# miaoyin390/DNN-Compression-Tensor-ADMM

Measured on AMD Instinct MI355X. Metric: ADMM projection iters/sec (all layers) + per-layer SVD GFLOP/s, ResNet-50 TT ranks, higher is better.
Workload: dtype f32 (Gram, eigen-solve and its filter products accumulate in f64); 1 GPU; resnet50_tt: 34 layers, 20099072 weights, hp table tt_resnet50_hp.HyperParamsDictGeneralRatio3x; tables=1, parallelism=layer-shard x1 (latency-model partition, one scalar all-reduce per step)

## Files before the change

### dnn-compression-tensor-admm_amd/csrc/common.h

```cpp
#pragma once
#include <hip/hip_runtime.h>
#include <stdint.h>
#include <stddef.h>
#include "../../include/tadmm.h"

namespace tadmm {

constexpr int kWave = 64;

struct BlockRef { int32_t prob; int32_t local; };

struct SweepDesc {
  const float* W; float* U; float* Z;
  float* T0;
  const float* Zmat;
  int32_t O, I, K2;
  int32_t ichunk;
  int32_t nchunk;
  int64_t numel;
  int32_t blk_begin;
  int32_t nblk;
};

void launch_unfold(const SweepDesc* descs_dev, const BlockRef* map_dev, int nblocks, int use_u, hipStream_t s);
void launch_fold_update(const SweepDesc* descs_dev, const BlockRef* map_dev, int nblocks, int update_u,
                        double* resid_partial_dev, hipStream_t s);
void launch_resid_reduce(const SweepDesc* descs_dev, int nlayers, const double* resid_partial_dev,
                         double* resid_sq_dev, hipStream_t s, const int32_t* out_index = nullptr);

struct GramDesc {
  const float* A;
  int32_t m, n;
  int32_t trans;
  int32_t N, K;
  int32_t nt;
  int32_t ksplit, kchunk;
  double* partial;
  double* G;
  int32_t Npad, ld;
};
void launch_gram_partial(const GramDesc* descs_dev, const BlockRef* map_dev, int nblocks, hipStream_t s,
                         const int32_t* skip = nullptr);
void launch_gram_reduce(const GramDesc* descs_dev, const BlockRef* map_dev, int nblocks, hipStream_t s,
                        const int32_t* skip = nullptr);

constexpr int kJB = 8;
struct EigDesc {
  double* XT;
  int32_t N, Npad, ld, nb;
  double* off;
  int32_t* done;
  double* lam;
  int32_t* order;
  double* sigma;
  int32_t r;
  int32_t mode;
  float* out_a;
  float* out_b;
  double* evec_out;
  double* sblk;
  int32_t ldo;
  double* warm;
  int32_t* warm_ok;
  double* scratch;
  int32_t period;
};
void launch_jacobi_init(const EigDesc* descs_dev, int nprob, hipStream_t s, const int32_t* skip = nullptr,
                        double* prev_dev = nullptr);
void launch_jacobi_conv(const EigDesc* descs_dev, int nprob, int tick, double tol, bool super, double* prev_dev,
                        int* verdict_pinned, hipStream_t s);
constexpr int kJacobiMaxN = 8160;
bool jacobi_size_supported(int n);
size_t jacobi_tick_stream_lds_bytes();
size_t jacobi_tick_lds_bytes(int ld_max);
size_t jacobi_tick2_lds_bytes(int ld_max);
bool jacobi_tick2_fits(int ld_max);
hipError_t launch_jacobi_tick(const EigDesc* descs_dev, const BlockRef* map_dev, int nblocks, int tick, double tol,
                              int inner_sweeps, size_t lds_bytes, bool super, hipStream_t s);
void dump_stamps();
size_t jacobi_tick3_lds_bytes(int ld_max);
bool jacobi_tick3_fits(int ld_max);
hipError_t launch_jacobi_tick3(const EigDesc* descs_dev, const BlockRef* map_dev, int nblocks, int tick, double tol,
                               int ld_max, hipStream_t s);
constexpr int kLdResidentMax = 1152;
static inline int eig_ld(int N) { return (N + 127) / 128 * 128; }
hipError_t launch_jacobi_self(const EigDesc* descs_dev, const BlockRef* map_dev, int nblocks, int tick, double tol,
                              int inner_sweeps, int ld_max, hipStream_t s);
bool jacobi_small_fits(int npad_max);
hipError_t launch_jacobi_small(const EigDesc* descs_dev, int nprob, int npad_max, double tol, int max_sweeps,
                               const int32_t* skip, int* verdict_pinned, hipStream_t s, bool warm,
                               const int32_t* fast_done = nullptr);
bool eig_small_direct_on();
bool eig_mid_direct_on();
bool eig_mid_direct_size(int n);
size_t eig_mid_scratch_bytes(int n);
void launch_eig_mid_direct(const EigDesc* descs_dev, int nprob, int ns, const int32_t* skip, int* verdict_pinned, hipStream_t s);
hipError_t launch_eig_small_direct(const EigDesc* descs_dev, int nprob, const int32_t* skip, int32_t* fast_done_dev,
                                   int* verdict_pinned, hipStream_t s);
void launch_eig_norms(const EigDesc* descs_dev, const BlockRef* map_dev, int nblocks, hipStream_t s,
                      const int32_t* skip = nullptr);
void launch_eig_sort(const EigDesc* descs_dev, int nprob, hipStream_t s, const int32_t* skip = nullptr, int npad_max = 0);
void launch_eig_extract(const EigDesc* descs_dev, const BlockRef* map_dev, int nblocks, hipStream_t s,
                        const int32_t* skip = nullptr);

struct GemmDesc {
  const float* A; const float* B; float* C;
  int32_t M, N, K;
  int64_t a_rs, a_cs, b_rs, b_cs, c_rs, c_cs;
  float alpha, beta;
  const float* bias_n; const float* bias_m;
  int32_t tiles_m, tiles_n;
};
constexpr int kGemmBM = 64, kGemmBN = 64;
void launch_gemm(const GemmDesc* descs_dev, const BlockRef* map_dev, int nblocks, hipStream_t s,
                 const int32_t* skip = nullptr);
void launch_gemm_one(const GemmDesc& d, hipStream_t s);
void launch_gemm_bf16_nt(const void* A, const void* Bt, void* C, int M, int N, int K, int64_t lda, int64_t ldb,
                         int64_t ldc, const float* bias_n, hipStream_t s);

#if defined(__HIP_DEVICE_COMPILE__) || defined(__HIPCC__)
template <typename T> using G = T __attribute__((address_space(1)));
template <typename T> __device__ __forceinline__ G<T>* gp(T* p) { return (G<T>*)p; }
#endif

struct ChainDesc {
  const void* X; void* Y;
  const uint16_t* Win; const uint16_t* Wout;
  const float* bias;
  int64_t T;
  int32_t Kin, R, Nout;
  int64_t ldx, ldy, win_plane, wout_plane;
  int32_t x_hw, y_hw, x_vec, y_vec, fused;
  long long* stamps;
  void* H;
  int64_t ldh;
  int32_t rt, h_vec;
};
int launch_tt_chain(const ChainDesc& d, int dtype, int tile_tokens, hipStream_t s);
int launch_svdconv_chain(const ChainDesc& d, int dtype, int tile_tokens, hipStream_t s);

struct ConvChainDesc {
  const void* X; void* Y;
  const uint16_t* W1; const uint16_t* W2; const uint16_t* W3;
  const float* bias;
  int64_t w1_plane, w2_plane, w3_plane;
  int32_t B, C, R1, R2, Nout;
  int32_t H, W, Ho, Wo, kh, kw, sh, sw, ph, pw, dh, dw;
  int32_t TM, TR, tiles, NT;
  int32_t x_vec;
  int32_t transposed;
  void* S1; void* S2;
  int32_t r1t, r2t;
};
int launch_tt_conv(const ConvChainDesc& d, int dtype, hipStream_t s);
bool plan_tt_conv(ConvChainDesc& d, int dtype, size_t* lds_bytes);

struct DgemmDesc {
  const double* A; const double* B; const double* C;
  const double* P; const double* Q;
  double* ring[3];
  const int32_t* rot;
  int32_t selA, selB, selC, selP, selQ;
  int32_t M, N, K;
  int32_t lda, ldb, ldc;
  int32_t tiles_m, tiles_n;
  int32_t mode;
  const double* coef;
  const double* theta;
  double* rowpart;
  const int32_t* gate; int32_t gate_min;
  const uint16_t* Gp; int64_t g_plane;
};
void launch_dgemm(const DgemmDesc* descs_dev, const BlockRef* map_dev, int nblocks, bool b_transposed, hipStream_t s);
void launch_dgemm_nt64(const DgemmDesc* descs_dev, const BlockRef* map_dev, int nblocks, hipStream_t s, int tile_n = 64,
                       int tile_m = 64);
void launch_daxpby(const DgemmDesc* descs_dev, const BlockRef* map_dev, int nblocks, hipStream_t s);
struct GPlaneDesc {
  const double* Gm; int32_t ldg;
  int32_t nt, ks;
  uint16_t* out; int64_t plane;
};
void launch_gplanes(const GPlaneDesc* descs_dev, const BlockRef* map_dev, int nblocks, hipStream_t s);
void launch_dgemm3(const DgemmDesc* descs_dev, const BlockRef* map_dev, int nblocks, hipStream_t s);

constexpr int kCholStrip = 16;
struct CholDesc {
  const double* C; int32_t ldc;
  int32_t n;
  double* R; int32_t ldr;
  double* Wd;
  double* ring[3]; const int32_t* rot; int32_t sel;
  int32_t ldy, ncols;
  int32_t* bad;
  const int32_t* gate; int32_t gate_min;
  int32_t* rot_out;
};
void launch_chol_factor(const CholDesc* descs_dev, int nprob, hipStream_t s);
void launch_chol_solve(const CholDesc* descs_dev, const BlockRef* map_dev, int nblocks, hipStream_t s);

struct FiltState {
  int32_t base, res;
  int32_t nsteps;
  int32_t active;
  int32_t alive;
  int32_t bad;
  int32_t stage;
  int32_t products;
  int32_t products_fast;
  int32_t precise_stages;
  double logamp;
  double logamp_precise;
  double coef1[2];
  double coefk[3];
  double b, lr, l1;
  double crit;
  double guard;
  double mom[64 * 5];
  int32_t mom_on;
};
struct FiltProb {
  FiltState* st;
  double* ring[3];
  int32_t N, Npad, rp, r, r32;
  int32_t ldy;
  const double* rqpart; int32_t rq_tiles;
  const double* vpart; int32_t v_tiles;
  const double* lam; const int32_t* order;
  double* sigma;
  double* theta;
  const double* UT;
  int32_t mode, ldo;
  float* out_a; float* out_b;
  int32_t* skip_slot;
  int32_t* fb_skip;
  const double* G; int32_t ldg;
  const double* H; int32_t ldh;
};
struct FiltParams {
  int32_t max_degree;
  double log_target;
  double cond_max;
  double cond_first;
  double sin_tol;
  double log_precise;
};
struct CompDesc {
  FiltState* st;
  const double* G; double* Gc;
  int32_t N, Npad, ldg;
  double* cshift;
  const double* UT; int32_t ldy, k;
  double* Cimg; int32_t r;
  float* out_a; int32_t ldo;
  double* sigma_layer;
};
void launch_comp_prepare(const CompDesc* descs_dev, int nprob, int npad_max, int steps, hipStream_t s);
void launch_comp_form(const CompDesc* descs_dev, const BlockRef* map_dev, int nblocks, hipStream_t s);
void launch_comp_emit(const CompDesc* descs_dev, const BlockRef* map_dev, int nblocks, hipStream_t s);
void launch_filt_init(const FiltProb* probs_dev, const BlockRef* map_dev, int nblocks, int nprob, hipStream_t s);
void launch_filt_guard(const FiltProb* probs_dev, int nprob, int npad_max, int rp_max, int steps, hipStream_t s);
void launch_filt_moments(const FiltProb* probs_dev, int nprob, hipStream_t s);
void launch_filt_plan(const FiltProb* probs_dev, int nprob, FiltParams prm, int last_stage, int stage_fast, int* verdict_pinned,
                      hipStream_t s);
void launch_filt_flags(const FiltProb* probs_dev, int nprob, hipStream_t s);
void launch_filt_theta(const FiltProb* probs_dev, int nprob, hipStream_t s);
void launch_filt_verdict(const FiltProb* probs_dev, int nprob, FiltParams prm, int* verdict_pinned, hipStream_t s);
void launch_filt_emit(const FiltProb* probs_dev, const BlockRef* map_dev, int nblocks, hipStream_t s);

constexpr int kPenaltyBlocks = 1024;
void launch_penalty(int n, const void* const* ptrs_dev, const int64_t* numel_dev, int64_t total, float rho,
                    float gscale, double* loss_dev, double* partial_dev, hipStream_t s);

}
```

### dnn-compression-tensor-admm_amd/csrc/gemm.hip

```cpp
#include "common.h"

namespace tadmm {

typedef float float16_t __attribute__((ext_vector_type(16)));

constexpr int BM = kGemmBM, BN = kGemmBN, BK = 16;
constexpr int LDA = BM + 4, LDB = BN + 4;

struct Frag4 { float v[4]; };

__device__ __forceinline__ Frag4 load_tile4(const float* __restrict__ P, int64_t rs, int64_t cs, bool kcontig,
                                            int row0, int nrows, int k0, int K, int tid) {
  Frag4 f;
  if (kcontig) {
    const int rr = tid >> 2, kk = (tid & 3) * 4;
    const int row = row0 + rr;
    const bool rok = row < nrows;
    const float* p = P + (int64_t)row * rs + (int64_t)(k0 + kk) * cs;
    if (rok && (k0 + kk + 3) < K && ((((uintptr_t)p) & 15) == 0)) {
      const float4 t = *reinterpret_cast<const float4*>(p);
      f.v[0] = t.x; f.v[1] = t.y; f.v[2] = t.z; f.v[3] = t.w;
    } else {
#pragma unroll
      for (int e = 0; e < 4; ++e) f.v[e] = (rok && (k0 + kk + e) < K) ? p[e] : 0.f;
    }
  } else {
    const int kk = tid >> 4, rr = (tid & 15) * 4;
    const int k = k0 + kk;
    const bool kok = k < K;
    const float* p = P + (int64_t)(row0 + rr) * rs + (int64_t)k * cs;
    if (kok && (row0 + rr + 3) < nrows && ((((uintptr_t)p) & 15) == 0)) {
      const float4 t = *reinterpret_cast<const float4*>(p);
      f.v[0] = t.x; f.v[1] = t.y; f.v[2] = t.z; f.v[3] = t.w;
    } else {
#pragma unroll
      for (int e = 0; e < 4; ++e) f.v[e] = (kok && (row0 + rr + e) < nrows) ? p[e] : 0.f;
    }
  }
  return f;
}

__device__ __forceinline__ void store_tile4(float* __restrict__ S, int ldS, bool kcontig, const Frag4& f, int tid) {
  if (kcontig) {
    const int rr = tid >> 2, kk = (tid & 3) * 4;
#pragma unroll
    for (int e = 0; e < 4; ++e) S[(kk + e) * ldS + rr] = f.v[e];
  } else {
    const int kk = tid >> 4, rr = (tid & 15) * 4;
    *reinterpret_cast<float4*>(&S[kk * ldS + rr]) = make_float4(f.v[0], f.v[1], f.v[2], f.v[3]);
  }
}

template <bool kComp>
__device__ __forceinline__ void gemm_tile(const GemmDesc& d, int local, float* __restrict__ As, float* __restrict__ Bs) {
  const int tm = local / d.tiles_n, tn = local - tm * d.tiles_n;
  const int m0 = tm * BM, n0 = tn * BN;
  const int tid = threadIdx.x, lane = tid & 63, wave = tid >> 6;
  const int wm = wave >> 1, wn = wave & 1;
  const bool a_k = (d.a_cs == 1), b_k = (d.b_rs == 1) && (d.b_cs != 1);
  const int K = d.K;
  const float16_t zero16 = {0, 0, 0, 0, 0, 0, 0, 0, 0, 0, 0, 0, 0, 0, 0, 0};
  float16_t acc0 = zero16, tot = zero16;

  Frag4 fa = load_tile4(d.A, d.a_rs, d.a_cs, a_k, m0, d.M, 0, K, tid);
  Frag4 fb = load_tile4(d.B, d.b_cs, d.b_rs, b_k, n0, d.N, 0, K, tid);
  const int ai = wm * 32 + (lane & 31), bj = wn * 32 + (lane & 31), kq = lane >> 5;
  int chunk = 0;
  for (int k0 = 0; k0 < K; k0 += BK) {
    store_tile4(As, LDA, a_k, fa, tid);
    store_tile4(Bs, LDB, b_k, fb, tid);
    __syncthreads();
    if (k0 + BK < K) {
      fa = load_tile4(d.A, d.a_rs, d.a_cs, a_k, m0, d.M, k0 + BK, K, tid);
      fb = load_tile4(d.B, d.b_cs, d.b_rs, b_k, n0, d.N, k0 + BK, K, tid);
    }
#pragma unroll
    for (int kk = 0; kk < BK; kk += 2) {
      const float a = As[(kk + kq) * LDA + ai];
      const float b = Bs[(kk + kq) * LDB + bj];
      acc0 = __builtin_amdgcn_mfma_f32_32x32x2f32(a, b, acc0, 0, 0, 0);
    }
    if (kComp && ++chunk == 4) {
      chunk = 0;
#pragma unroll
      for (int e = 0; e < 16; ++e) tot[e] += acc0[e];
      acc0 = zero16;
    }
    __syncthreads();
  }
  float16_t acc;
#pragma unroll
  for (int e = 0; e < 16; ++e) acc[e] = kComp ? tot[e] + acc0[e] : acc0[e];

  const int col = n0 + wn * 32 + (lane & 31);
  if (col < d.N) {
    const float bn = d.bias_n ? d.bias_n[col] : 0.f;
#pragma unroll
    for (int reg = 0; reg < 16; ++reg) {
      const int row = m0 + wm * 32 + (reg & 3) + 8 * (reg >> 2) + 4 * (lane >> 5);
      if (row < d.M) {
        float* c = d.C + (int64_t)row * d.c_rs + (int64_t)col * d.c_cs;
        float v = d.alpha * acc[reg] + bn;
        if (d.bias_m) v += d.bias_m[row];
        if (d.beta != 0.f) v += d.beta * (*c);
        *c = v;
      }
    }
  }
}

template <bool kComp>
__global__ __launch_bounds__(256) void gemm_kernel(const GemmDesc* __restrict__ descs,
                                                   const BlockRef* __restrict__ map,
                                                   const int32_t* __restrict__ skip) {
  __shared__ __attribute__((aligned(16))) float As[BK * LDA];
  __shared__ __attribute__((aligned(16))) float Bs[BK * LDB];
  const BlockRef br = map[blockIdx.x];
  if (skip && skip[br.prob]) return;
  const GemmDesc d = descs[br.prob];
  gemm_tile<kComp>(d, br.local, As, Bs);
}

template <bool kComp>
__global__ __launch_bounds__(256) void gemm_one_kernel(const GemmDesc d) {
  __shared__ __attribute__((aligned(16))) float As[BK * LDA];
  __shared__ __attribute__((aligned(16))) float Bs[BK * LDB];
  gemm_tile<kComp>(d, blockIdx.x, As, Bs);
}

static bool gemm_plain() {
  const char* e = getenv("TADMM_GEMM_PLAIN");
  return e && atoi(e);
}

void launch_gemm_one(const GemmDesc& d, hipStream_t s) {
  const int nblocks = d.tiles_m * d.tiles_n;
  if (nblocks <= 0) return;
  if (gemm_plain()) hipLaunchKernelGGL(gemm_one_kernel<false>, dim3(nblocks), dim3(256), 0, s, d);
  else hipLaunchKernelGGL(gemm_one_kernel<true>, dim3(nblocks), dim3(256), 0, s, d);
}

void launch_gemm(const GemmDesc* descs_dev, const BlockRef* map_dev, int nblocks, hipStream_t s, const int32_t* skip) {
  if (nblocks <= 0) return;
  if (gemm_plain()) hipLaunchKernelGGL(gemm_kernel<false>, dim3(nblocks), dim3(256), 0, s, descs_dev, map_dev, skip);
  else hipLaunchKernelGGL(gemm_kernel<true>, dim3(nblocks), dim3(256), 0, s, descs_dev, map_dev, skip);
}

}
```

### dnn-compression-tensor-admm_amd/csrc/gram.hip

```cpp
#include "common.h"

namespace tadmm {

typedef double double4_t __attribute__((ext_vector_type(4)));

__device__ __forceinline__ double4_t mfma_f64(double a, double b, double4_t c) {
  return __builtin_amdgcn_mfma_f64_16x16x4f64(a, b, c, 0, 0, 0);
}

__device__ __forceinline__ void tile_pair(int tp, int nt, int& ti, int& tj) {
  int a = 0, rowlen = nt;
  while (tp >= rowlen) { tp -= rowlen; ++a; --rowlen; }
  ti = a; tj = a + tp;
}

__global__ __launch_bounds__(256) void gram_partial_kernel(const GramDesc* __restrict__ descs,
                                                           const BlockRef* __restrict__ map,
                                                           const int32_t* __restrict__ skip) {
  __shared__ double red[4][4][64 * 4];
  __shared__ double tile[32][33];
  const BlockRef br = map[blockIdx.x];
  if (skip && skip[br.prob]) return;
  const GramDesc d = descs[br.prob];
  const int ntp = d.nt * (d.nt + 1) / 2;
  const int ks = br.local / ntp;
  const int tp = br.local - ks * ntp;
  int ti, tj;
  tile_pair(tp, d.nt, ti, tj);
  const bool diag = (ti == tj);
  const int lane = threadIdx.x & 63, wave = threadIdx.x >> 6;
  const int r = lane & 15, q = lane >> 4;

  const int kbeg = ks * d.kchunk;
  const int kend = min(d.K, kbeg + d.kchunk);
  const int per = (((kend - kbeg + 3) / 4) + 15) & ~15;
  const int wk0 = min(kend, kbeg + wave * per);
  const int wk1 = min(kend, wk0 + per);

  double4_t acc00 = {0, 0, 0, 0}, acc01 = {0, 0, 0, 0}, acc10 = {0, 0, 0, 0}, acc11 = {0, 0, 0, 0};
  const float* A = d.A;
  const int N = d.N;
  const int ra0 = ti * 32 + r, ra1 = ra0 + 16;
  const int rb0 = tj * 32 + r, rb1 = rb0 + 16;
  const float ma0 = ra0 < N ? 1.f : 0.f, ma1 = ra1 < N ? 1.f : 0.f;
  const float mb0 = rb0 < N ? 1.f : 0.f, mb1 = rb1 < N ? 1.f : 0.f;
  const int64_t ld = d.n;

  struct Chunk { float a0[4], a1[4], b0[4], b1[4]; };
  auto mma = [&](const Chunk& c) {
#pragma unroll
    for (int e = 0; e < 4; ++e) {
      const double da0 = c.a0[e], da1 = c.a1[e];
      const double db0 = diag ? da0 : (double)c.b0[e], db1 = diag ? da1 : (double)c.b1[e];
      acc00 = mfma_f64(da0, db0, acc00);
      acc01 = mfma_f64(da0, db1, acc01);
      if (!diag) acc10 = mfma_f64(da1, db0, acc10);
      acc11 = mfma_f64(da1, db1, acc11);
    }
  };

  if (!d.trans) {
    const bool vec = ((ld & 3) == 0) && ((((uintptr_t)A) & 15) == 0);
    const float* pa0 = A + (int64_t)min(ra0, N - 1) * ld;
    const float* pa1 = A + (int64_t)min(ra1, N - 1) * ld;
    const float* pb0 = A + (int64_t)min(rb0, N - 1) * ld;
    const float* pb1 = A + (int64_t)min(rb1, N - 1) * ld;
    auto fetch = [&](int kk, Chunk& c) {
      const int k = kk + 4 * q;
      if (vec && k + 3 < wk1) {
        const float4 t0 = *reinterpret_cast<const float4*>(pa0 + k);
        const float4 t1 = *reinterpret_cast<const float4*>(pa1 + k);
        c.a0[0] = t0.x * ma0; c.a0[1] = t0.y * ma0; c.a0[2] = t0.z * ma0; c.a0[3] = t0.w * ma0;
        c.a1[0] = t1.x * ma1; c.a1[1] = t1.y * ma1; c.a1[2] = t1.z * ma1; c.a1[3] = t1.w * ma1;
        if (!diag) {
          const float4 t2 = *reinterpret_cast<const float4*>(pb0 + k);
          const float4 t3 = *reinterpret_cast<const float4*>(pb1 + k);
          c.b0[0] = t2.x * mb0; c.b0[1] = t2.y * mb0; c.b0[2] = t2.z * mb0; c.b0[3] = t2.w * mb0;
          c.b1[0] = t3.x * mb1; c.b1[1] = t3.y * mb1; c.b1[2] = t3.z * mb1; c.b1[3] = t3.w * mb1;
        }
      } else {
#pragma unroll
        for (int e = 0; e < 4; ++e) {
          const bool ok = (k + e) < wk1;
          c.a0[e] = ok ? pa0[k + e] * ma0 : 0.f;
          c.a1[e] = ok ? pa1[k + e] * ma1 : 0.f;
          c.b0[e] = (ok && !diag) ? pb0[k + e] * mb0 : 0.f;
          c.b1[e] = (ok && !diag) ? pb1[k + e] * mb1 : 0.f;
        }
      }
    };
    if (wk0 < wk1) {
      Chunk cur, nxt;
      fetch(wk0, cur);
      for (int kk = wk0; kk < wk1; kk += 16) {
        const bool more = kk + 16 < wk1;
        if (more) fetch(kk + 16, nxt);
        mma(cur);
        if (more) cur = nxt;
      }
    }
  } else {
    const int ca0 = min(ra0, N - 1), ca1 = min(ra1, N - 1), cb0 = min(rb0, N - 1), cb1 = min(rb1, N - 1);
    auto fetch = [&](int kk, Chunk& c) {
#pragma unroll
      for (int e = 0; e < 4; ++e) {
        const int k = kk + 4 * e + q;
        const bool ok = k < wk1;
        const float* row = A + (int64_t)min(k, d.K - 1) * ld;
        c.a0[e] = ok ? row[ca0] * ma0 : 0.f;
        c.a1[e] = ok ? row[ca1] * ma1 : 0.f;
        c.b0[e] = (ok && !diag) ? row[cb0] * mb0 : 0.f;
        c.b1[e] = (ok && !diag) ? row[cb1] * mb1 : 0.f;
      }
    };
    if (wk0 < wk1) {
      Chunk cur, nxt;
      fetch(wk0, cur);
      for (int kk = wk0; kk < wk1; kk += 16) {
        const bool more = kk + 16 < wk1;
        if (more) fetch(kk + 16, nxt);
        mma(cur);
        if (more) cur = nxt;
      }
    }
  }

#pragma unroll
  for (int e = 0; e < 4; ++e) {
    red[wave][0][lane * 4 + e] = acc00[e];
    red[wave][1][lane * 4 + e] = acc01[e];
    red[wave][2][lane * 4 + e] = acc10[e];
    red[wave][3][lane * 4 + e] = acc11[e];
  }
  __syncthreads();
  if (d.ksplit > 1) {
    double* out = d.partial + ((int64_t)ks * ntp + tp) * 1024;
    for (int idx = threadIdx.x; idx < 1024; idx += 256) {
      const int t = idx >> 8, le = idx & 255;
      const double v = (red[0][t][le] + red[1][t][le]) + (red[2][t][le] + red[3][t][le]);
      const int l = le >> 2, reg = le & 3;
      const int row = (t >> 1) * 16 + (l >> 4) + 4 * reg;
      const int col = (t & 1) * 16 + (l & 15);
      out[row * 32 + col] = v;
    }
    return;
  }
  for (int idx = threadIdx.x; idx < 1024; idx += 256) {
    const int t = idx >> 8, le = idx & 255;
    if (diag && t == 2) continue;
    const double v = (red[0][t][le] + red[1][t][le]) + (red[2][t][le] + red[3][t][le]);
    const int l = le >> 2, reg = le & 3;
    const int row = (t >> 1) * 16 + (l >> 4) + 4 * reg;
    const int col = (t & 1) * 16 + (l & 15);
    tile[row][col] = v;
    if (diag && t == 1) tile[col][row] = v;
  }
  __syncthreads();
  double* __restrict__ G = d.G;
  const int64_t gld = d.ld;
  for (int e = threadIdx.x; e < 1024; e += 256) {
    const int rr = e >> 5, cc = e & 31;
    G[(int64_t)(ti * 32 + rr) * gld + tj * 32 + cc] = tile[rr][cc];
    if (!diag) G[(int64_t)(tj * 32 + rr) * gld + ti * 32 + cc] = tile[cc][rr];
  }
  if (tj == d.nt - 1) {
    const int padw = d.ld - d.Npad;
    for (int e = threadIdx.x; e < 32 * padw; e += 256) {
      const int rr = e / padw, cc = e - rr * padw;
      G[(int64_t)(ti * 32 + rr) * gld + d.Npad + cc] = 0.0;
    }
  }
}

__global__ __launch_bounds__(256) void gram_reduce_kernel(const GramDesc* __restrict__ descs,
                                                          const BlockRef* __restrict__ map,
                                                          const int32_t* __restrict__ skip) {
  const BlockRef br = map[blockIdx.x];
  if (skip && skip[br.prob]) return;
  const GramDesc d = descs[br.prob];
  const int ntp = d.nt * (d.nt + 1) / 2;
  const int64_t total = (int64_t)d.Npad * d.ld;
  const int64_t base = (int64_t)br.local * 1024;
  for (int t = threadIdx.x; t < 1024; t += 256) {
    const int64_t idx = base + t;
    if (idx >= total) break;
    const int j = (int)(idx / d.ld), i = (int)(idx - (int64_t)j * d.ld);
    double v = 0.0;
    if (j < d.N && i < d.N) {
      int a = j >> 5, b = i >> 5, jr = j & 31, ir = i & 31;
      if (a > b) { int s = a; a = b; b = s; s = jr; jr = ir; ir = s; }
      if (a == b && jr > ir) { const int s = jr; jr = ir; ir = s; }
      const int tp = a * d.nt - (a * (a - 1)) / 2 + (b - a);
      const double* p = d.partial + (int64_t)tp * 1024 + jr * 32 + ir;
      const int64_t stride = (int64_t)ntp * 1024;
      int ks = 0;
      for (; ks + 8 <= d.ksplit; ks += 8) {
        double t[8];
#pragma unroll
        for (int u = 0; u < 8; ++u) t[u] = p[(ks + u) * stride];
        v += ((t[0] + t[1]) + (t[2] + t[3])) + ((t[4] + t[5]) + (t[6] + t[7]));
      }
      for (; ks < d.ksplit; ++ks) v += p[ks * stride];
    }
    d.G[idx] = v;
  }
}

void launch_gram_partial(const GramDesc* descs_dev, const BlockRef* map_dev, int nblocks, hipStream_t s,
                         const int32_t* skip) {
  if (nblocks <= 0) return;
  hipLaunchKernelGGL(gram_partial_kernel, dim3(nblocks), dim3(256), 0, s, descs_dev, map_dev, skip);
}

void launch_gram_reduce(const GramDesc* descs_dev, const BlockRef* map_dev, int nblocks, hipStream_t s,
                        const int32_t* skip) {
  if (nblocks <= 0) return;
  hipLaunchKernelGGL(gram_reduce_kernel, dim3(nblocks), dim3(256), 0, s, descs_dev, map_dev, skip);
}

}
```

Measured before the change: 164.4 iters/s.

## Deepen prefetch pipelines in f32 GEMM and f64 Gram kernels with specialized loaders

The GEMM kernel moves to BK=32 with double-buffered shared memory, a multi-stage register prefetch, and templated tile loaders chosen per layout (k-contiguous, row-contiguous, edge) that clamp row indices instead of branching. The Gram partial kernel gets compile-time diag/trans specialization, a deeper register prefetch ring (3-4 chunks), unaligned vector loads through global address-space pointers, and a separate tail path. Both aim to hide global-load latency and cut per-iteration bounds checks. The cost is higher register and LDS pressure and more template instantiations, which may lower occupancy. The Kahan-style fold cadence in the GEMM also changes, which can shift rounding slightly.

```diff
diff --git a/dnn-compression-tensor-admm_amd/csrc/common.h b/dnn-compression-tensor-admm_amd/csrc/common.h
--- a/dnn-compression-tensor-admm_amd/csrc/common.h
+++ b/dnn-compression-tensor-admm_amd/csrc/common.h
@@ -121,6 +121,7 @@
 #if defined(__HIP_DEVICE_COMPILE__) || defined(__HIPCC__)
 template <typename T> using G = T __attribute__((address_space(1)));
 template <typename T> __device__ __forceinline__ G<T>* gp(T* p) { return (G<T>*)p; }
+typedef float f4u __attribute__((ext_vector_type(4), aligned(4)));
 #endif
 
 struct ChainDesc {
diff --git a/dnn-compression-tensor-admm_amd/csrc/gemm.hip b/dnn-compression-tensor-admm_amd/csrc/gemm.hip
--- a/dnn-compression-tensor-admm_amd/csrc/gemm.hip
+++ b/dnn-compression-tensor-admm_amd/csrc/gemm.hip
@@ -4,93 +4,208 @@
 
 typedef float float16_t __attribute__((ext_vector_type(16)));
 
-constexpr int BM = kGemmBM, BN = kGemmBN, BK = 16;
+constexpr int BM = kGemmBM, BN = kGemmBN;
+constexpr int BK = 32;
 constexpr int LDA = BM + 4, LDB = BN + 4;
-
-struct Frag4 { float v[4]; };
-
-__device__ __forceinline__ Frag4 load_tile4(const float* __restrict__ P, int64_t rs, int64_t cs, bool kcontig,
-                                            int row0, int nrows, int k0, int K, int tid) {
-  Frag4 f;
-  if (kcontig) {
-    const int rr = tid >> 2, kk = (tid & 3) * 4;
-    const int row = row0 + rr;
-    const bool rok = row < nrows;
-    const float* p = P + (int64_t)row * rs + (int64_t)(k0 + kk) * cs;
-    if (rok && (k0 + kk + 3) < K && ((((uintptr_t)p) & 15) == 0)) {
-      const float4 t = *reinterpret_cast<const float4*>(p);
-      f.v[0] = t.x; f.v[1] = t.y; f.v[2] = t.z; f.v[3] = t.w;
+constexpr int kStage = BK * (LDA + LDB);
+constexpr int NPF = 2;
+
+enum : int { kKc = 0, kRc = 1, kRe = 2 };
+
+struct Frag8 { float v[2][4]; };
+
+template <int MODE>
+struct TileLoader {
+  const G<const float>* base;
+  int64_t rowoff[4];
+  int64_t cs;
+  int kk;
+
+  __device__ __forceinline__ void init(const float* P, int64_t rs, int64_t cs_, int row0, int nrows, int tid) {
+    base = gp(P);
+    if (MODE == kKc) {
+      kk = (tid & 3) * 4; cs = 1;
+      rowoff[0] = (int64_t)min(row0 + (tid >> 2), nrows - 1) * rs;
+      rowoff[1] = rowoff[2] = rowoff[3] = 0;
     } else {
-#pragma unroll
-      for (int e = 0; e < 4; ++e) f.v[e] = (rok && (k0 + kk + e) < K) ? p[e] : 0.f;
-    }
-  } else {
-    const int kk = tid >> 4, rr = (tid & 15) * 4;
-    const int k = k0 + kk;
-    const bool kok = k < K;
-    const float* p = P + (int64_t)(row0 + rr) * rs + (int64_t)k * cs;
-    if (kok && (row0 + rr + 3) < nrows && ((((uintptr_t)p) & 15) == 0)) {
-      const float4 t = *reinterpret_cast<const float4*>(p);
-      f.v[0] = t.x; f.v[1] = t.y; f.v[2] = t.z; f.v[3] = t.w;
-    } else {
-#pragma unroll
-      for (int e = 0; e < 4; ++e) f.v[e] = (kok && (row0 + rr + e) < nrows) ? p[e] : 0.f;
-    }
-  }
-  return f;
-}
-
-__device__ __forceinline__ void store_tile4(float* __restrict__ S, int ldS, bool kcontig, const Frag4& f, int tid) {
-  if (kcontig) {
-    const int rr = tid >> 2, kk = (tid & 3) * 4;
-#pragma unroll
-    for (int e = 0; e < 4; ++e) S[(kk + e) * ldS + rr] = f.v[e];
-  } else {
-    const int kk = tid >> 4, rr = (tid & 15) * 4;
-    *reinterpret_cast<float4*>(&S[kk * ldS + rr]) = make_float4(f.v[0], f.v[1], f.v[2], f.v[3]);
-  }
+      kk = tid >> 4; cs = cs_;
+      const int rr = (tid & 15) * 4;
+#pragma unroll
+      for (int e = 0; e < 4; ++e) rowoff[e] = min(row0 + rr + e, nrows - 1);
+    }
+  }
+  __device__ __forceinline__ void load(Frag8& f, int k0) const {
+#pragma unroll
+    for (int j = 0; j < 2; ++j) {
+      const int k = k0 + 16 * j + kk;
+      if (MODE == kRe) {
+#pragma unroll
+        for (int e = 0; e < 4; ++e) f.v[j][e] = base[(int64_t)k * cs + rowoff[e]];
+      } else {
+        const G<const float>* p = (MODE == kKc) ? base + rowoff[0] + k : base + (int64_t)k * cs + rowoff[0];
+        const f4u t = *reinterpret_cast<const G<const f4u>*>(p);
+        f.v[j][0] = t.x; f.v[j][1] = t.y; f.v[j][2] = t.z; f.v[j][3] = t.w;
+      }
+    }
+  }
+  __device__ __forceinline__ void load_tail(Frag8& f, int k0, int K) const {
+#pragma unroll
+    for (int j = 0; j < 2; ++j) {
+      if (MODE == kRc) {
+        const f4u t = *reinterpret_cast<const G<const f4u>*>(base + (int64_t)min(k0 + 16 * j + kk, K - 1) * cs + rowoff[0]);
+        f.v[j][0] = t.x; f.v[j][1] = t.y; f.v[j][2] = t.z; f.v[j][3] = t.w;
+        continue;
+      }
+#pragma unroll
+      for (int e = 0; e < 4; ++e) {
+        const int k = k0 + 16 * j + kk + (MODE == kKc ? e : 0);
+        const int kc = min(k, K - 1);
+        f.v[j][e] = (MODE == kKc) ? base[rowoff[0] + kc] : base[(int64_t)kc * cs + rowoff[e]];
+      }
+    }
+  }
+  __device__ __forceinline__ void zero_tail(Frag8& f, int k0, int K) const {
+#pragma unroll
+    for (int j = 0; j < 2; ++j) {
+#pragma unroll
+      for (int e = 0; e < 4; ++e) {
+        const int k = k0 + 16 * j + kk + (MODE == kKc ? e : 0);
+        f.v[j][e] = (k < K) ? f.v[j][e] : 0.f;
+      }
+    }
+  }
+  __device__ __forceinline__ void store(float* __restrict__ S, int ldS, const Frag8& f, int tid) const {
+#pragma unroll
+    for (int j = 0; j < 2; ++j) {
+      if (MODE == kKc) {
+        const int rr = tid >> 2;
+#pragma unroll
+        for (int e = 0; e < 4; ++e) S[(16 * j + kk + e) * ldS + rr] = f.v[j][e];
+      } else {
+        const int rr = (tid & 15) * 4;
+        *reinterpret_cast<float4*>(&S[(16 * j + kk) * ldS + rr]) = make_float4(f.v[j][0], f.v[j][1], f.v[j][2], f.v[j][3]);
+      }
+    }
+  }
+};
+
+template <bool kComp, int AMODE, int BMODE>
+__device__ __forceinline__ float16_t gemm_tile_sum(const GemmDesc& d, int m0, int n0, float* __restrict__ smem) {
+  static_assert(NPF % 2 == 0, "the fold follows the odd stages of the unrolled loop");
+  const int tid = threadIdx.x, lane = tid & 63, wave = tid >> 6;
+  const int wm = wave >> 1, wn = wave & 1;
+  const int K = d.K;
+  const int nfull = K / BK, rem = K - nfull * BK;
+  TileLoader<AMODE> la;
+  TileLoader<BMODE> lb;
+  la.init(d.A, d.a_rs, d.a_cs, m0, d.M, tid);
+  lb.init(d.B, d.b_cs, d.b_rs, n0, d.N, tid);
+
+  const float16_t zero16 = {0, 0, 0, 0, 0, 0, 0, 0, 0, 0, 0, 0, 0, 0, 0, 0};
+  float16_t acc0 = zero16, tot = zero16;
+  const int ai = wm * 32 + (lane & 31), bj = wn * 32 + (lane & 31), kq = lane >> 5;
+  auto sstore = [&](const Frag8& fa, const Frag8& fb, int stage) {
+    float* As = smem + stage * kStage;
+    la.store(As, LDA, fa, tid);
+    lb.store(As + BK * LDA, LDB, fb, tid);
+  };
+  auto compute = [&](int stage) {
+    const float* As = smem + stage * kStage;
+    const float* Bs = As + BK * LDA;
+    float a[BK / 2], b[BK / 2];
+#pragma unroll
+    for (int s = 0; s < BK / 2; ++s) {
+      a[s] = As[(2 * s + kq) * LDA + ai];
+      b[s] = Bs[(2 * s + kq) * LDB + bj];
+    }
+    __builtin_amdgcn_sched_barrier(0);
+#pragma unroll
+    for (int s = 0; s < BK / 2; ++s) acc0 = __builtin_amdgcn_mfma_f32_32x32x2f32(a[s], b[s], acc0, 0, 0, 0);
+  };
+  auto compute_half = [&](int stage, int h) {
+    const float* As = smem + stage * kStage + 16 * h * LDA;
+    const float* Bs = smem + stage * kStage + BK * LDA + 16 * h * LDB;
+    float a[BK / 4], b[BK / 4];
+#pragma unroll
+    for (int s = 0; s < BK / 4; ++s) {
+      a[s] = As[(2 * s + kq) * LDA + ai];
+      b[s] = Bs[(2 * s + kq) * LDB + bj];
+    }
+#pragma unroll
+    for (int s = 0; s < BK / 4; ++s) acc0 = __builtin_amdgcn_mfma_f32_32x32x2f32(a[s], b[s], acc0, 0, 0, 0);
+  };
+  auto fold = [&]() {
+#pragma unroll
+    for (int e = 0; e < 16; ++e) tot[e] += acc0[e];
+    acc0 = zero16;
+  };
+
+  Frag8 ta, tb;
+  if (rem) {
+    la.load_tail(ta, nfull * BK, K);
+    lb.load_tail(tb, nfull * BK, K);
+  }
+  Frag8 ra[NPF], rb[NPF];
+  if (nfull > 0) {
+    const int last = nfull - 1;
+#pragma unroll
+    for (int u = 0; u < NPF; ++u) { la.load(ra[u], min(u, last) * BK); lb.load(rb[u], min(u, last) * BK); }
+    sstore(ra[0], rb[0], 0);
+    la.load(ra[0], min(NPF, last) * BK);
+    lb.load(rb[0], min(NPF, last) * BK);
+    __syncthreads();
+    int c = 0;
+    for (; c + NPF <= nfull; c += NPF) {
+#pragma unroll
+      for (int u = 0; u < NPF; ++u) {
+        const int i = c + u;
+        if (i + 1 < nfull) sstore(ra[(u + 1) % NPF], rb[(u + 1) % NPF], (u + 1) & 1);
+        la.load(ra[(u + 1) % NPF], min(i + 1 + NPF, last) * BK);
+        lb.load(rb[(u + 1) % NPF], min(i + 1 + NPF, last) * BK);
+        __builtin_amdgcn_sched_barrier(0);
+        compute(u & 1);
+        if (kComp && (u & 1)) fold();
+        __syncthreads();
+      }
+    }
+    if (c < nfull) {
+      compute(0);
+      __syncthreads();
+    }
+  }
+  if (rem) {
+    la.zero_tail(ta, nfull * BK, K);
+    lb.zero_tail(tb, nfull * BK, K);
+    sstore(ta, tb, nfull & 1);
+    __syncthreads();
+    compute_half(nfull & 1, 0);
+    if (rem > 16) compute_half(nfull & 1, 1);
+    if (kComp && (nfull & 1) && rem > 16) fold();
+  }
+  float16_t acc;
+#pragma unroll
+  for (int e = 0; e < 16; ++e) acc[e] = kComp ? tot[e] + acc0[e] : acc0[e];
+  return acc;
 }
 
 template <bool kComp>
-__device__ __forceinline__ void gemm_tile(const GemmDesc& d, int local, float* __restrict__ As, float* __restrict__ Bs) {
+__device__ __forceinline__ void gemm_tile(const GemmDesc& d, int local, float* __restrict__ smem) {
   const int tm = local / d.tiles_n, tn = local - tm * d.tiles_n;
   const int m0 = tm * BM, n0 = tn * BN;
   const int tid = threadIdx.x, lane = tid & 63, wave = tid >> 6;
   const int wm = wave >> 1, wn = wave & 1;
   const bool a_k = (d.a_cs == 1), b_k = (d.b_rs == 1) && (d.b_cs != 1);
-  const int K = d.K;
-  const float16_t zero16 = {0, 0, 0, 0, 0, 0, 0, 0, 0, 0, 0, 0, 0, 0, 0, 0};
-  float16_t acc0 = zero16, tot = zero16;
-
-  Frag4 fa = load_tile4(d.A, d.a_rs, d.a_cs, a_k, m0, d.M, 0, K, tid);
-  Frag4 fb = load_tile4(d.B, d.b_cs, d.b_rs, b_k, n0, d.N, 0, K, tid);
-  const int ai = wm * 32 + (lane & 31), bj = wn * 32 + (lane & 31), kq = lane >> 5;
-  int chunk = 0;
-  for (int k0 = 0; k0 < K; k0 += BK) {
-    store_tile4(As, LDA, a_k, fa, tid);
-    store_tile4(Bs, LDB, b_k, fb, tid);
-    __syncthreads();
-    if (k0 + BK < K) {
-      fa = load_tile4(d.A, d.a_rs, d.a_cs, a_k, m0, d.M, k0 + BK, K, tid);
-      fb = load_tile4(d.B, d.b_cs, d.b_rs, b_k, n0, d.N, k0 + BK, K, tid);
-    }
-#pragma unroll
-    for (int kk = 0; kk < BK; kk += 2) {
-      const float a = As[(kk + kq) * LDA + ai];
-      const float b = Bs[(kk + kq) * LDB + bj];
-      acc0 = __builtin_amdgcn_mfma_f32_32x32x2f32(a, b, acc0, 0, 0, 0);
-    }
-    if (kComp && ++chunk == 4) {
-      chunk = 0;
-#pragma unroll
-      for (int e = 0; e < 16; ++e) tot[e] += acc0[e];
-      acc0 = zero16;
-    }
-    __syncthreads();
-  }
+  const int am = a_k ? kKc : (m0 + BM <= d.M ? kRc : kRe);
+  const int bm = b_k ? kKc : (n0 + BN <= d.N ? kRc : kRe);
   float16_t acc;
-#pragma unroll
-  for (int e = 0; e < 16; ++e) acc[e] = kComp ? tot[e] + acc0[e] : acc0[e];
+#define TADMM_GEMM_CASE(A_, B_) case A_ * 3 + B_: acc = gemm_tile_sum<kComp, A_, B_>(d, m0, n0, smem); break;
+  switch (am * 3 + bm) {
+    TADMM_GEMM_CASE(kKc, kKc) TADMM_GEMM_CASE(kKc, kRc) TADMM_GEMM_CASE(kKc, kRe)
+    TADMM_GEMM_CASE(kRc, kKc) TADMM_GEMM_CASE(kRc, kRc) TADMM_GEMM_CASE(kRc, kRe)
+    TADMM_GEMM_CASE(kRe, kKc) TADMM_GEMM_CASE(kRe, kRc)
+    default: acc = gemm_tile_sum<kComp, kRe, kRe>(d, m0, n0, smem); break;
+  }
+#undef TADMM_GEMM_CASE
 
   const int col = n0 + wn * 32 + (lane & 31);
   if (col < d.N) {
@@ -113,24 +228,22 @@
 __global__ __launch_bounds__(256) void gemm_kernel(const GemmDesc* __restrict__ descs,
                                                    const BlockRef* __restrict__ map,
                                                    const int32_t* __restrict__ skip) {
-  __shared__ __attribute__((aligned(16))) float As[BK * LDA];
-  __shared__ __attribute__((aligned(16))) float Bs[BK * LDB];
+  __shared__ __attribute__((aligned(16))) float smem[2 * kStage];
   const BlockRef br = map[blockIdx.x];
   if (skip && skip[br.prob]) return;
   const GemmDesc d = descs[br.prob];
-  gemm_tile<kComp>(d, br.local, As, Bs);
+  gemm_tile<kComp>(d, br.local, smem);
 }
 
 template <bool kComp>
 __global__ __launch_bounds__(256) void gemm_one_kernel(const GemmDesc d) {
-  __shared__ __attribute__((aligned(16))) float As[BK * LDA];
-  __shared__ __attribute__((aligned(16))) float Bs[BK * LDB];
-  gemm_tile<kComp>(d, blockIdx.x, As, Bs);
+  __shared__ __attribute__((aligned(16))) float smem[2 * kStage];
+  gemm_tile<kComp>(d, blockIdx.x, smem);
 }
 
 static bool gemm_plain() {
-  const char* e = getenv("TADMM_GEMM_PLAIN");
-  return e && atoi(e);
+  static const bool plain = getenv("TADMM_GEMM_PLAIN") && atoi(getenv("TADMM_GEMM_PLAIN"));
+  return plain;
 }
 
 void launch_gemm_one(const GemmDesc& d, hipStream_t s) {
diff --git a/dnn-compression-tensor-admm_amd/csrc/gram.hip b/dnn-compression-tensor-admm_amd/csrc/gram.hip
--- a/dnn-compression-tensor-admm_amd/csrc/gram.hip
+++ b/dnn-compression-tensor-admm_amd/csrc/gram.hip
@@ -1,4 +1,5 @@
 #include "common.h"
+#include <type_traits>
 
 namespace tadmm {
 
@@ -28,7 +29,7 @@
   int ti, tj;
   tile_pair(tp, d.nt, ti, tj);
   const bool diag = (ti == tj);
-  const int lane = threadIdx.x & 63, wave = threadIdx.x >> 6;
+  const int lane = threadIdx.x & 63, wave = __builtin_amdgcn_readfirstlane(threadIdx.x >> 6);
   const int r = lane & 15, q = lane >> 4;
 
   const int kbeg = ks * d.kchunk;
@@ -38,92 +39,102 @@
   const int wk1 = min(kend, wk0 + per);
 
   double4_t acc00 = {0, 0, 0, 0}, acc01 = {0, 0, 0, 0}, acc10 = {0, 0, 0, 0}, acc11 = {0, 0, 0, 0};
-  const float* A = d.A;
+  const G<const float>* A = gp(d.A);
   const int N = d.N;
   const int ra0 = ti * 32 + r, ra1 = ra0 + 16;
   const int rb0 = tj * 32 + r, rb1 = rb0 + 16;
   const float ma0 = ra0 < N ? 1.f : 0.f, ma1 = ra1 < N ? 1.f : 0.f;
   const float mb0 = rb0 < N ? 1.f : 0.f, mb1 = rb1 < N ? 1.f : 0.f;
   const int64_t ld = d.n;
+  const int ca0 = min(ra0, N - 1), ca1 = min(ra1, N - 1), cb0 = min(rb0, N - 1), cb1 = min(rb1, N - 1);
 
   struct Chunk { float a0[4], a1[4], b0[4], b1[4]; };
-  auto mma = [&](const Chunk& c) {
-#pragma unroll
-    for (int e = 0; e < 4; ++e) {
-      const double da0 = c.a0[e], da1 = c.a1[e];
-      const double db0 = diag ? da0 : (double)c.b0[e], db1 = diag ? da1 : (double)c.b1[e];
-      acc00 = mfma_f64(da0, db0, acc00);
-      acc01 = mfma_f64(da0, db1, acc01);
-      if (!diag) acc10 = mfma_f64(da1, db0, acc10);
-      acc11 = mfma_f64(da1, db1, acc11);
-    }
+  const int nfull =(wk1 - wk0) >> 4, rem = (wk1 - wk0) & 15;
+  const int ktail = wk0 + 16 * nfull;
+  auto body = [&](auto diag_tag, auto trans_tag) {
+    constexpr bool kDiag = decltype(diag_tag)::value, kTrans = decltype(trans_tag)::value;
+    constexpr int NPF = kTrans ? 3 : 4;
+    auto mma = [&](const Chunk& c) {
+#pragma unroll
+      for (int e = 0; e < 4; ++e) {
+        const double da0 = c.a0[e], da1 = c.a1[e];
+        const double db0 = kDiag ? da0 : (double)c.b0[e], db1 = kDiag ? da1 : (double)c.b1[e];
+        acc00 = mfma_f64(da0, db0, acc00);
+        acc01 = mfma_f64(da0, db1, acc01);
+        if (!kDiag) acc10 = mfma_f64(da1, db0, acc10);
+        acc11 = mfma_f64(da1, db1, acc11);
+      }
+    };
+    auto cook = [&](const Chunk& c, bool tail) {
+      Chunk o;
+#pragma unroll
+      for (int e = 0; e < 4; ++e) {
+        const bool ok = !tail || (ktail + (kTrans ? 4 * e + q : 4 * q + e)) < wk1;
+        o.a0[e] = ok ? c.a0[e] * ma0 : 0.f;
+        o.a1[e] = ok ? c.a1[e] * ma1 : 0.f;
+        o.b0[e] = (ok && !kDiag) ? c.b0[e] * mb0 : 0.f;
+        o.b1[e] = (ok && !kDiag) ? c.b1[e] * mb1 : 0.f;
+      }
+      return o;
+    };
+    const G<const float>* pa0 = A + (kTrans ? (int64_t)ca0 : (int64_t)ca0 * ld);
+    const G<const float>* pa1 = A + (kTrans ? (int64_t)ca1 : (int64_t)ca1 * ld);
+    const G<const float>* pb0 = A + (kTrans ? (int64_t)cb0 : (int64_t)cb0 * ld);
+    const G<const float>* pb1 = A + (kTrans ? (int64_t)cb1 : (int64_t)cb1 * ld);
+    auto ld4 = [&](float (&o)[4], const G<const float>* p) {
+      const f4u t = *reinterpret_cast<const G<const f4u>*>(p);
+      o[0] = t.x; o[1] = t.y; o[2] = t.z; o[3] = t.w;
+    };
+    auto fetch = [&](Chunk& c, int kk) {
+      if (!kTrans) {
+        const int k = kk + 4 * q;
+        ld4(c.a0, pa0 + k); ld4(c.a1, pa1 + k);
+        if (!kDiag) { ld4(c.b0, pb0 + k); ld4(c.b1, pb1 + k); }
+      } else {
+#pragma unroll
+        for (int e = 0; e < 4; ++e) {
+          const int64_t ro = (int64_t)(kk + 4 * e + q) * ld;
+          c.a0[e] = pa0[ro]; c.a1[e] = pa1[ro];
+          if (!kDiag) { c.b0[e] = pb0[ro]; c.b1[e] = pb1[ro]; }
+        }
+      }
+    };
+    auto fetch_tail = [&](Chunk& c) {
+#pragma unroll
+      for (int e = 0; e < 4; ++e) {
+        const int kc = min(ktail + (kTrans ? 4 * e + q : 4 * q + e), wk1 - 1);
+        const int64_t o = kTrans ? (int64_t)kc * ld : (int64_t)kc;
+        c.a0[e] = pa0[o]; c.a1[e] = pa1[o];
+        if (!kDiag) { c.b0[e] = pb0[o]; c.b1[e] = pb1[o]; }
+      }
+    };
+    Chunk tail = {};
+    if (rem) fetch_tail(tail);
+    if (nfull > 0) {
+      const int last = nfull - 1;
+      Chunk R[NPF] = {};
+#pragma unroll
+      for (int u = 0; u < NPF; ++u) fetch(R[u], wk0 + 16 * min(u, last));
+      int c = 0;
+      for (; c + NPF <= nfull; c += NPF) {
+#pragma unroll
+        for (int u = 0; u < NPF; ++u) {
+          const Chunk cur = cook(R[u], false);
+          fetch(R[u], wk0 + 16 * min(c + u + NPF, last));
+          __builtin_amdgcn_sched_barrier(0);
+          mma(cur);
+        }
+      }
+#pragma unroll
+      for (int u = 0; u < NPF - 1; ++u)
+        if (c + u < nfull) mma(cook(R[u], false));
+    }
+    if (rem) mma(cook(tail, true));
   };
-
-  if (!d.trans) {
-    const bool vec = ((ld & 3) == 0) && ((((uintptr_t)A) & 15) == 0);
-    const float* pa0 = A + (int64_t)min(ra0, N - 1) * ld;
-    const float* pa1 = A + (int64_t)min(ra1, N - 1) * ld;
-    const float* pb0 = A + (int64_t)min(rb0, N - 1) * ld;
-    const float* pb1 = A + (int64_t)min(rb1, N - 1) * ld;
-    auto fetch = [&](int kk, Chunk& c) {
-      const int k = kk + 4 * q;
-      if (vec && k + 3 < wk1) {
-        const float4 t0 = *reinterpret_cast<const float4*>(pa0 + k);
-        const float4 t1 = *reinterpret_cast<const float4*>(pa1 + k);
-        c.a0[0] = t0.x * ma0; c.a0[1] = t0.y * ma0; c.a0[2] = t0.z * ma0; c.a0[3] = t0.w * ma0;
-        c.a1[0] = t1.x * ma1; c.a1[1] = t1.y * ma1; c.a1[2] = t1.z * ma1; c.a1[3] = t1.w * ma1;
-        if (!diag) {
-          const float4 t2 = *reinterpret_cast<const float4*>(pb0 + k);
-          const float4 t3 = *reinterpret_cast<const float4*>(pb1 + k);
-          c.b0[0] = t2.x * mb0; c.b0[1] = t2.y * mb0; c.b0[2] = t2.z * mb0; c.b0[3] = t2.w * mb0;
-          c.b1[0] = t3.x * mb1; c.b1[1] = t3.y * mb1; c.b1[2] = t3.z * mb1; c.b1[3] = t3.w * mb1;
-        }
-      } else {
-#pragma unroll
-        for (int e = 0; e < 4; ++e) {
-          const bool ok = (k + e) < wk1;
-          c.a0[e] = ok ? pa0[k + e] * ma0 : 0.f;
-          c.a1[e] = ok ? pa1[k + e] * ma1 : 0.f;
-          c.b0[e] = (ok && !diag) ? pb0[k + e] * mb0 : 0.f;
-          c.b1[e] = (ok && !diag) ? pb1[k + e] * mb1 : 0.f;
-        }
-      }
-    };
-    if (wk0 < wk1) {
-      Chunk cur, nxt;
-      fetch(wk0, cur);
-      for (int kk = wk0; kk < wk1; kk += 16) {
-        const bool more = kk + 16 < wk1;
-        if (more) fetch(kk + 16, nxt);
-        mma(cur);
-        if (more) cur = nxt;
-      }
-    }
-  } else {
-    const int ca0 = min(ra0, N - 1), ca1 = min(ra1, N - 1), cb0 = min(rb0, N - 1), cb1 = min(rb1, N - 1);
-    auto fetch = [&](int kk, Chunk& c) {
-#pragma unroll
-      for (int e = 0; e < 4; ++e) {
-        const int k = kk + 4 * e + q;
-        const bool ok = k < wk1;
-        const float* row = A + (int64_t)min(k, d.K - 1) * ld;
-        c.a0[e] = ok ? row[ca0] * ma0 : 0.f;
-        c.a1[e] = ok ? row[ca1] * ma1 : 0.f;
-        c.b0[e] = (ok && !diag) ? row[cb0] * mb0 : 0.f;
-        c.b1[e] = (ok && !diag) ? row[cb1] * mb1 : 0.f;
-      }
-    };
-    if (wk0 < wk1) {
-      Chunk cur, nxt;
-      fetch(wk0, cur);
-      for (int kk = wk0; kk < wk1; kk += 16) {
-        const bool more = kk + 16 < wk1;
-        if (more) fetch(kk + 16, nxt);
-        mma(cur);
-        if (more) cur = nxt;
-      }
-    }
-  }
+  using T = std::true_type;
+  using F = std::false_type;
+  if (!d.trans) { if (diag) body(T(), F()); else body(F(), F()); }
+  else          { if (diag) body(T(), T()); else body(F(), T()); }
 
 #pragma unroll
   for (int e = 0; e < 4; ++e) {
```

Measured after the change: 169.0 iters/s (median of 6 runs). 1.03x the previous value.
